# syncdoth/face_mask_inpaint

Measured on AMD Instinct MI355X. Metric: train images/sec at 256x256 bs=8 per GPU (PICNet-ref train step), higher is better.
Workload: dtype f32; 1 GPU; train_reference_fill.py PICNet-ref 256x256 fp32, bs=8 per GPU, synthetic CelebA-HQ-shaped batch + random binary_map (BASELINE configs[1]); global_batch=8, parallelism=dp1

## Files before the change

face_mask_inpaint_amd/_lib.py:

```python
from __future__ import annotations

import ctypes as C
import os

_HERE = os.path.dirname(os.path.abspath(__file__))
LIB_PATH = os.path.join(_HERE, "csrc", "libfmi_hip.so")

c_f = C.c_void_p
i32, i64, f32, f64, vp = C.c_int, C.c_int64, C.c_float, C.c_double, C.c_void_p


class ConvDesc(C.Structure):

    _fields_ = [(n, C.c_int) for n in ("N", "H", "W", "C", "OH", "OW", "K", "x_cstride", "y_cstride", "kh", "kw", "stride", "pad", "pad_mode", "dil")] + [("w3", C.c_void_p), ("x3", C.c_void_p), ("y3", C.c_void_p)]


class WeightEntry(C.Structure):
    _fields_ = [("w", vp), ("u", vp), ("v", vp), ("wf", vp), ("wt", vp), ("sigma", vp), ("rows", i32), ("C", i32), ("taps", i32), ("iters", i32), ("wf3", vp), ("wt3", vp)]


class WeightGradEntry(C.Structure):
    _fields_ = [("w", vp), ("u", vp), ("v", vp), ("sigma", vp), ("dwf", vp), ("dw", vp), ("rows", i32), ("C", i32), ("taps", i32), ("pad_", i32)]


class AdamEntry(C.Structure):
    _fields_ = [("p", vp), ("g", vp), ("m", vp), ("v", vp), ("n", i64)]


class RangerEntry(C.Structure):
    _fields_ = [("p", vp), ("g", vp), ("m", vp), ("v", vp), ("slow", vp), ("row_mean", vp), ("n", i64), ("cols", i64)]


PD = C.POINTER(ConvDesc)

SIGNATURES = {
    "fmi_gemm_f32": [vp, vp, vp, i32, i32, i32, i64, i64, i64, i64, i64, i64, i32, i64, i64, i64, f32, f32, vp, vp],
    "fmi_ssim_valid_f32": [vp, vp, vp, i32, i32, i32, i32, f32, f32, vp, vp, i64, vp],
    "fmi_avgpool2_pad_f32": [vp, vp, i32, i32, i32, i32, i32, vp],
    "fmi_resample_u8": [vp, vp, i32, i32, i32, i32, i32, i32, i32, i32, vp, vp, i32, vp],
    "fmi_gather_u8_i64": [vp, vp, i32, i32, i32, i32, i32, vp, vp, vp],
    "fmi_u8_lut_chw_f32": [vp, vp, vp, i32, i32, i32, i32, vp],
    "fmi_split3_f32": [vp, vp, vp, i64, i32, i32, f32, vp],
    "fmi_split3_colsum_f32": [vp, vp, vp, i64, i32, vp],
    "fmi_merge3_f32": [vp, vp, i64, i32, vp],
    "fmi_conv2d_fwd_f32": [PD, vp, vp, vp, vp, vp, i32, i32, i64, vp],
    "fmi_conv2d_dgrad_f32": [PD, vp, vp, vp, vp, vp, i32, i64, vp],
    "fmi_conv_transpose2d_pair_f32": [PD, vp, vp, i32, vp, vp, vp, vp],
    "fmi_conv_transpose2d_pair_bwd_f32": [PD, vp, vp, i32, vp, vp, vp, vp, vp, vp, vp, vp, vp, i64, vp],
    "fmi_conv2d_pair_fwd_f32": [PD, vp, vp, i32, vp, vp, vp, vp, vp, vp, i32, vp],
    "fmi_conv2d_pair_wgrad_f32": [PD, vp, vp, i32, vp, vp, vp, vp, vp],
    "fmi_conv2d_dgrad_masked_f32": [PD, vp, vp, vp, f32, vp, vp],
    "fmi_conv2d_dgrad_masked_add_f32": [PD, vp, vp, vp, f32, vp, vp, vp],
    "fmi_conv2d_wgrad_f32": [PD, vp, vp, vp, vp, i32, i64, vp],
    "fmi_conv2d_thin_fwd_f32": [PD, vp, vp, vp, vp, vp, i32, vp],
    "fmi_conv2d_thin_dgrad_f32": [PD, vp, vp, vp, vp],
    "fmi_conv2d_thin_input_dgrad_f32": [PD, vp, vp, vp, vp],
    "fmi_conv2d_thin_in_fwd_f32": [PD, vp, vp, vp, vp, vp, i32, vp],
    "fmi_conv2d_thin_in_wgrad_f32": [PD, vp, vp, vp, vp, vp, i64, vp],
    "fmi_conv2d_thin_lrelu_fwd_f32": [PD, vp, f32, vp, vp, vp, i32, vp],
    "fmi_conv2d_thin_lrelu_fwd_bf16": [PD, vp, f32, vp, vp, vp, i32, vp],
    "fmi_conv2d_thin_lrelu_dgrad_f32": [PD, vp, vp, vp, f32, vp, vp],
    "fmi_conv2d_thin_lrelu_wgrad_f32": [PD, vp, f32, vp, vp, vp, vp],
    "fmi_conv2d_thin_wgrad_f32": [PD, vp, vp, vp, vp, vp],
    "fmi_conv2d_thin_lrelu_bwd_f32": [PD, vp, f32, vp, vp, vp, vp, vp, vp, vp, i64, vp],
    "fmi_conv2d_fwd_bf16": [PD, vp, vp, vp, vp, vp, i64, vp],
    "fmi_conv2d_dgrad_bf16": [PD, vp, vp, vp, vp, vp, i64, vp],
    "fmi_conv2d_wgrad_bf16": [PD, vp, vp, vp, vp],
    "fmi_pack_weight_bf16": [vp, vp, i32, i32, i32, vp],
    "fmi_scale_channels_bf16": [vp, vp, vp, i32, i64, i32, vp],
    "fmi_scale_channels_gs_bf16": [vp, vp, vp, vp, i64, i32, i64, i32, vp],
    "fmi_noise_bias_act_bf16": [vp, vp, vp, vp, vp, i64, i32, f32, f32, vp],
    "fmi_noise_bias_act_bwd_bf16": [vp, vp, vp, vp, vp, vp, vp, i64, i64, i32, f32, f32, vp],
    "fmi_upfirdn2d_nhwc_bf16": [vp, vp, vp] + [i32] * 14 + [vp],
    "fmi_styled_out_bwd_bf16": [vp] * 11 + [i64, vp, i32, i64, i32, f32, f32, vp],
    "fmi_conv2d_fwd_act_bf16": [PD, vp, vp, vp, vp, vp, vp, f32, f32, vp, vp],
    "fmi_conv2d_fwd_chan_bf16": [PD, vp, vp, vp, vp, vp, vp, vp, i64, vp],
    "fmi_se_gate_f32": [vp, i32, i64, f32, vp, vp, vp, i32, i32, vp],
    "fmi_irse_tail_bf16": [vp] * 8 + [i32] * 7 + [vp],
    "fmi_irse_stem_bf16": [vp] * 5 + [i64, i32, vp],
    "fmi_conv2d_grouped_fwd_bf16": [PD, i32, i64, vp, vp, vp, f32, vp, vp, vp],
    "fmi_fpn_merge_bf16": [vp] * 4 + [i32] * 6 + [vp],
    "fmi_conv2d_thin_in_fwd_bf16": [PD, vp, vp, vp, f32, vp, vp],
    "fmi_irse_stem_fwd_bf16": [PD] + [vp] * 11,
    "fmi_fpn_merge_in_bf16": [vp] * 3 + [i32] * 6 + [vp],
    "fmi_mask_blend_bf16": [vp] * 4 + [i64, i32, vp],
    "fmi_conv2d_c32_fwd_bf16": [PD, vp, vp, vp, f32, vp, vp],
    "fmi_conv2d_dgrad_relu_bf16": [PD, vp, vp, vp, vp, vp],
    "fmi_vgg_tap_fwd_bf16": [vp, vp, vp, i32, i32, i32, i32, vp],
    "fmi_vgg_tap_bwd_bf16": [vp, vp, vp, vp, i32, i32, i32, i32, vp],
    "fmi_conv2d_thin_input_dgrad_bf16": [PD, vp, vp, vp, vp],
    "fmi_resblock_tail_bf16": [vp] * 5 + [i32] * 5 + [f32, vp],
    "fmi_picnet_stem_tail_bf16": [vp] * 6 + [i32] * 5 + [f32, vp],
    "fmi_guided_attention_fwd_bf16": [vp] * 5 + [i32] * 5 + [vp],
    "fmi_guided_attention_sliced_fwd_bf16": [vp] * 5 + [i32] * 5 + [vp],
    "fmi_blur_act_bf16": [vp, vp, vp] + [i32] * 8 + [vp, vp, vp, vp, f32, f32, i32, vp],
    "fmi_torgb_fwd_bf16": [vp, vp, vp, vp, vp, vp, i32, i64, i32, vp],
    "fmi_torgb_bwd_bf16": [vp, vp, vp, vp, vp, vp, i64, vp, vp, vp, i32, i64, i32, vp],
    "fmi_bias_grad_f32": [vp, i64, i32, i32, vp, vp],
    "fmi_reflect_pad_fold_f32": [vp, vp, i32, i32, i32, i32, i32, vp],
    "fmi_weight_prepare_f32": [vp, i32, vp],
    "fmi_weight_grad_f32": [vp, i32, vp, vp],
    "fmi_softmax_rows_f32": [vp, vp, i64, i32, vp],
    "fmi_softmax_rows_bwd_f32": [vp, vp, vp, i64, i32, vp],
    "fmi_attention_fwd_f32": [vp, vp, vp, vp, vp, vp, i32, i32, i32, i32, i32, vp],
    "fmi_attention_fwd_bf16": [vp] * 6 + [i32] * 5 + [vp],
    "fmi_attention_bwd_f32": [vp] * 12 + [i32] * 5 + [vp],
    "fmi_attention_bwd_prep_bf16": [vp] * 4 + [i32] * 4 + [vp],
    "fmi_attention_bwd_bf16": [vp] * 7 + [i32] * 4 + [vp],
    "fmi_attention_fwd_image_bytes": [i32, i32, i32, i32, i32, C.POINTER(i64)],
    "fmi_attention_fwd_pieces_f32": [vp] * 4 + [i64] + [vp] * 3 + [i32] * 5 + [vp],
    "fmi_attention_bwd_image_bytes": [i32, i32, i32, i32, i32, C.POINTER(i64)],
    "fmi_attention_bwd_pieces_f32": [vp] * 10 + [i64] + [vp] * 3 + [i32] * 5 + [vp],
    "fmi_eltwise_f32": [i32, vp, vp, vp, i64, f32, vp],
    "fmi_axpy_dev_f32": [vp, vp, vp, vp, i64, vp],
    "fmi_dot_f32": [vp, vp, i64, f32, vp, vp],
    "fmi_mask_binarise_i64": [vp, vp, i64, vp],
    "fmi_mask_mul_f32": [vp, vp, vp, i64, i32, i32, vp],
    "fmi_guide_blend_f32": [vp, vp, vp, vp, i64, i32, i32, vp],
    "fmi_guide_blend_bwd_f32": [vp, vp, vp, vp, i64, i32, i32, vp],
    "fmi_vae_sample_f32": [vp, vp, vp, vp, vp, i64, i32, vp],
    "fmi_vae_sample_bwd_f32": [vp, vp, vp, vp, vp, vp, vp, i64, i32, vp],
    "fmi_avgpool_f32": [vp, vp, i32, i32, i32, i32, i32, vp],
    "fmi_avgpool_bwd_f32": [vp, vp, i32, i32, i32, i32, i32, vp],
    "fmi_maxpool2_f32": [vp, vp, i32, i32, i32, i32, vp],
    "fmi_maxpool2_bf16": [vp, vp, i32, i32, i32, i32, vp],
    "fmi_maxpool2_bwd_bf16": [vp, vp, vp, i32, i32, i32, i32, vp],
    "fmi_up2_cat_bf16": [vp, vp, vp, i32, i32, i32, i32, i32, i32, i32, vp],
    "fmi_up2_cat_bwd_bf16": [vp, vp, vp, i32, i32, i32, i32, i32, i32, i32, vp],
    "fmi_head1x1_bf16": [vp, vp, vp, vp, i64, i32, i32, vp],
    "fmi_head1x1_argmax_bf16": [vp, vp, vp, vp, i64, i32, i32, vp],
    "fmi_head1x1_bwd_bf16": [vp, vp, vp, vp, vp, vp, vp, i64, i64, i32, i32, vp],
    "fmi_adaptive_avgpool_f32": [vp, vp, i32, i32, i32, i32, i32, i32, vp],
    "fmi_adaptive_avgpool_bwd_f32": [vp, vp, i32, i32, i32, i32, i32, i32, vp],
    "fmi_maxpool_f32": [vp, vp, vp, i32, i32, i32, i32, i32, i32, vp],
    "fmi_maxpool_bwd_f32": [vp, vp, vp, i32, i32, i32, i32, i32, i32, vp],
    "fmi_argmax_channels_f32": [vp, vp, i64, i32, vp],
    "fmi_image_tail_f32": [vp, vp, vp, vp, i32, i32, f32, f32, vp],
    "fmi_planes_to_u8_f32": [vp, vp, i32, i32, i32, i32, f32, f32, vp],
    "fmi_instnorm_stats_bf16": [vp, vp, vp, i32, i32, i32, f32, vp, i64, vp],
    "fmi_instnorm_apply_bf16": [vp, vp, vp, vp, vp, i32, i32, i32, f32, vp],
    "fmi_instnorm_bwd_reduce_bf16": [vp, vp, vp, vp, vp, vp, i32, i32, i32, f32, vp, i64, vp],
    "fmi_instnorm_bwd_apply_bf16": [vp, vp, vp, vp, vp, vp, vp, vp, vp, vp, i32, i32, i32, f32, vp],
    "fmi_prelu_bf16": [vp, vp, vp, i64, i32, vp],
    "fmi_prelu_bwd_bf16": [vp, vp, vp, vp, vp, vp, i64, i64, i32, vp],
    "fmi_scale_channels_add_bf16": [vp, vp, vp, vp, i32, i64, i32, vp],
    "fmi_add_bf16": [vp, vp, vp, i64, vp],
    "fmi_global_avgpool_bf16": [vp, vp, vp, i64, i32, i64, i32, vp],
    "fmi_add_bcast_bf16": [vp, vp, vp, i32, i64, i32, vp],
    "fmi_add_bcast_f32": [vp, vp, vp, i32, i64, i32, vp],
    "fmi_scale_channels_bwd_f32": [vp, vp, vp, vp, vp, vp, i64, i32, i64, i32, vp],
    "fmi_subsample_bf16": [vp, vp, i32, i32, i32, i32, i32, i32, vp],
    "fmi_scale_channels_add_f32": [vp, vp, vp, vp, i32, i64, i32, vp],
    "fmi_instnorm_bwd_apply_add_f32": [vp, vp, vp, vp, vp, vp, vp, vp, vp, vp, i32, i32, i32, f32, vp],
    "fmi_copy_channels_f32": [vp, vp, i64, i32, i32, i32, i32, i32, vp],
    "fmi_copy_channels_bf16": [vp, vp, i64, i32, i32, i32, i32, i32, vp],
    "fmi_l2norm_rows_f32": [vp, vp, vp, i64, i32, f32, vp],
    "fmi_l2norm_rows_bwd_f32": [vp, vp, vp, vp, i64, i32, f32, vp],
    "fmi_lpips_layer_f32": [vp, vp, vp, vp, i64, i32, f32, vp],
    "fmi_lpips_layer_bwd_f32": [vp, vp, vp, vp, vp, vp, i64, i32, f32, vp],
    "fmi_maxpool2_bwd_f32": [vp, vp, vp, i32, i32, i32, i32, vp],
    "fmi_resize_bilinear_f32": [vp, vp, i32, i32, i32, i32, i32, i32, vp, vp, vp],
    "fmi_resize_bilinear_bwd_f32": [vp, vp, i32, i32, i32, i32, i32, i32, vp, vp],
    "fmi_instnorm_stats_f32": [vp, vp, vp, i32, i32, i32, f32, vp, i64, vp],
    "fmi_batchnorm_running_update_f32": [vp, vp, vp, vp, vp, i32, i64, f32, f32, vp],
    "fmi_batchnorm_running_update_offset_f32": [vp, vp, vp, vp, vp, vp, i32, i64, f32, f32, vp],
    "fmi_instnorm_apply_f32": [vp, vp, vp, vp, vp, i32, i32, i32, f32, vp],
    "fmi_instnorm_bwd_reduce_f32": [vp, vp, vp, vp, vp, vp, i32, i32, i32, f32, vp, i64, vp],
    "fmi_instnorm_bwd_apply_f32": [vp, vp, vp, vp, vp, vp, vp, vp, vp, i32, i32, i32, f32, vp],
    "fmi_reduce_loss_f32": [i32, vp, vp, i64, f32, f32, vp, vp],
    "fmi_reduce_loss_bwd_f32": [i32, vp, vp, i64, f32, f32, vp, vp, vp],
    "fmi_ssim_f32": [vp, vp, vp, i32, i32, i32, i32, i32, vp, vp],
    "fmi_seg_ce_dice_fwd_f32": [vp, vp, i32, i64, i32, f64, vp, vp, vp, i64, vp],
    "fmi_seg_ce_dice_bwd_f32": [vp, vp, i32, i64, i32, f64, vp, vp, vp, vp],
# ... 97 lines not shown
```

face_mask_inpaint_amd/functional.py:

```python
from __future__ import annotations

import ctypes as C
import math
from typing import List, Optional, Sequence, Tuple

import torch

from . import _lib
from ._lib import ConvDesc, FmiError

EW_LRELU, EW_LRELU_BWD, EW_TANH_BWD, EW_ADD, EW_SCALE, EW_AXPY, EW_MUL, EW_RELU_BWD_OUT, EW_SOFTPLUS, EW_SOFTPLUS_BWD, EW_SUB, EW_RSQRT, EW_RSQRT_BWD, EW_SIGMOID, EW_SIGMOID_BWD = range(15)
ACT_NONE, ACT_TANH, ACT_RELU = 0, 1, 2

ATTN_CHUNK_BYTES = 96 * 1024 * 1024

PROFILE = None


class _prof:
    def __init__(self, tag, flops):
        self.tag, self.flops = tag, flops

    def __enter__(self):
        if PROFILE is not None:
# ... 1657 lines not shown
                d, a, prof = _conv_fwd_bf16_pre(hmap, k, 3, 3, 1, 1, " thin-in +relu")
                with prof:
                    lib.conv2d_thin_in_fwd_bf16(C.byref(d), _p(hmap), _p(wf), _p(bias), 0.0, _p(a), _st())
            elif _vgg_fwd_entry(c, k) == "chan":
                a = conv2d_chan_bf16(hmap, wnk, 3, 3, 1, 1, bias=bias, slope=zslope)
            else:
                d, a, prof = _conv_fwd_bf16_pre(hmap, k, 3, 3, 1, 1, " +relu")
                with prof:
                    lib.conv2d_fwd_act_bf16(C.byref(d), _p(hmap), _p(wnk), None, None, None, _p(bias), 0.0, 1.0, _p(a), _st())
            acts.append(a)
            hmap = a
            li += 1
        n, h, w, c = hmap.shape
        tap = torch.empty((n, h, w, c), device=x.device, dtype=torch.float32)
        pooled = torch.empty((n, h // 2, w // 2, c), device=x.device, dtype=BF16) if bi + 1 < len(blocks) else None
        with _prof(f"vgg_tap_fwd_bf16|{n}x{h}x{w}x{c}" + ("" if pooled is None else " +pool"), 0.0):
            lib.vgg_tap_fwd_bf16(_p(hmap), _p(tap), _p(pooled), n, h, w, c, _st())
        taps.append(tap)
        hmap = pooled
    return taps, acts


class _VggTrunkBF16(torch.autograd.Function):

    @staticmethod
    def forward(ctx, x, packs, blocks):
        taps, acts = _vgg_trunk_fwd(x, packs, blocks)
        ctx.save_for_backward(*acts)
        ctx.packs, ctx.blocks = packs, blocks
        ctx.set_materialize_grads(False)
        return tuple(taps)

    @staticmethod
    def backward(ctx, *gtaps):
        lib = _L()
        acts, packs, blocks = ctx.saved_tensors, ctx.packs, ctx.blocks
        first = [sum(blocks[:bi]) for bi in range(len(blocks))]
        gpool = None
        for bi in reversed(range(len(blocks))):
            last = first[bi] + blocks[bi] - 1
            a = acts[last]
            n, h, w, k = a.shape
            if gtaps[bi] is None and gpool is None:
                continue
            gt = torch.zeros((n, h, w, k), device=a.device, dtype=torch.float32) if gtaps[bi] is None else gtaps[bi].contiguous()
            _chk(gt)
            dy = torch.empty_like(a)
            with _prof(f"vgg_tap_bwd_bf16|{n}x{h}x{w}x{k}" + ("" if gpool is None else " +unpool"), 0.0):
                lib.vgg_tap_bwd_bf16(_p(a), _p(gt), _p(gpool), _p(dy), n, h, w, k, _st())
            for li in range(last, first[bi] - 1, -1):
                _wf, wt, _wnk, wck, _bias, _z = packs[li]
                k, c = wt.shape[1], wt.shape[2]
                d, _, _ = conv_desc(n, h, w, c, k, 3, 3, 1, 1)
                flops = 2.0 * dy.numel() * c * 9
                if li == 0:
                    gx = torch.empty((n, h, w, c), device=dy.device, dtype=torch.float32)
                    with _prof(f"conv_dgrad_bf16|{n}x{h}x{w} {c}->{k} k3s1 thin-in", flops):
                        lib.conv2d_thin_input_dgrad_bf16(C.byref(d), _p(dy), _p(wt), _p(gx), _st())
                    return gx, None, None
                dx = torch.empty((n, h, w, c), device=dy.device, dtype=BF16)
                if li > first[bi]:
                    with _prof(f"conv_dgrad_bf16|{n}x{h}x{w} {c}->{k} k3s1 +mask", flops):
                        lib.conv2d_dgrad_relu_bf16(C.byref(d), _p(dy), _p(wck), _p(acts[li - 1]), _p(dx), _st())
                else:
                    with _prof(f"conv_dgrad_bf16|{n}x{h}x{w} {c}->{k} k3s1", flops):
                        lib.conv2d_dgrad_bf16(C.byref(d), _p(dy), _p(wck), None, _p(dx), None, 0, _st())
                dy = dx
            gpool = dy
        return None, None, None


def vgg_trunk_bf16(x, packs, blocks=(2, 2, 3, 3)):
    if x.dim() != 4 or x.shape[3] > 4:
        raise FmiError(f"the bf16 VGG trunk takes an NHWC image with at most 4 channels, got {tuple(x.shape)}")
    vgg_trunk_check_extent(x.shape[1], x.shape[2])
    _chk(x)
    if len(packs) != sum(blocks):
        raise FmiError(f"the bf16 VGG trunk has {sum(blocks)} convolutions, got {len(packs)} packs")
    if torch.is_grad_enabled() and x.requires_grad:
        return list(_VggTrunkBF16.apply(x, packs, tuple(blocks)))
    return _vgg_trunk_fwd(x, packs, tuple(blocks))[0]


class _Resize(torch.autograd.Function):
    @staticmethod
    def forward(ctx, x, oh, ow, mean, std):
        _chk(x, mean, std)
        n, h, w, c = x.shape
        y = torch.empty((n, oh, ow, c), device=x.device, dtype=torch.float32)
        _L().resize_bilinear_f32(_p(x), _p(y), n, h, w, c, oh, ow, _p(mean), _p(std), _st())
        ctx.shape, ctx.std = x.shape, std
        return y

    @staticmethod
    def backward(ctx, g):
        n, h, w, c = ctx.shape
        gx = _zeros(ctx.shape, g.device, torch.float32)
        _L().resize_bilinear_bwd_f32(_p(g.contiguous()), _p(gx), n, h, w, c, g.shape[1], g.shape[2], _p(ctx.std), _st())
        return gx, None, None, None, None


def resize_bilinear(x, oh, ow, mean=None, std=None):
    return _Resize.apply(x, oh, ow, mean, std)


def _norm_ws(device, n, c):
    sums = torch.empty((n, c, 2), device=device, dtype=torch.float64)
    ws = torch.empty(max(1024, n) * c * 2, device=device, dtype=torch.float64)
    return sums, ws


class _InstNormAct(torch.autograd.Function):
    @staticmethod
    def forward(ctx, x, gamma, beta, eps, slope, passthrough=False):
        _chk(x, gamma, beta)
        lib = _L()
        n, h, w, c = x.shape
        sums, ws = _norm_ws(x.device, n, c)
        stats = torch.empty((n, c, 2), device=x.device, dtype=torch.float32)
        lib.instnorm_stats_f32(_p(x), C.c_void_p(sums.data_ptr()), _p(stats), n, h * w, c, eps, C.c_void_p(ws.data_ptr()), ws.numel(), _st())
        y = torch.empty_like(x)
        lib.instnorm_apply_f32(_p(x), _p(stats), _p(gamma), _p(beta), _p(y), n, h * w, c, slope, _st())
        ctx.save_for_backward(x, stats, gamma, beta)
        ctx.slope = slope
        if passthrough:
            return y, x.view_as(x)
        return y

    @staticmethod
    def backward(ctx, g, gpass=None):
        lib = _L()
        x, stats, gamma, beta = ctx.saved_tensors
        if g is None:
            return gpass, None, None, None, None, None
        n, h, w, c = x.shape
        g = g.contiguous()
        red, ws = _norm_ws(x.device, n, c)
        lib.instnorm_bwd_reduce_f32(_p(x), _p(g), _p(stats), _p(gamma), _p(beta), C.c_void_p(red.data_ptr()), n, h * w, c, ctx.slope,
                                    C.c_void_p(ws.data_ptr()), ws.numel(), _st())
        gx = torch.empty_like(x)
        dg = _zeros_like(gamma)
        db = _zeros_like(beta)
        if gpass is not None:
            lib.instnorm_bwd_apply_add_f32(_p(x), _p(g), _p(stats), _p(gamma), _p(beta), C.c_void_p(red.data_ptr()), _p(gpass.contiguous()),
                                           _p(gx), _p(dg), _p(db), n, h * w, c, ctx.slope, _st())
        else:
            lib.instnorm_bwd_apply_f32(_p(x), _p(g), _p(stats), _p(gamma), _p(beta), C.c_void_p(red.data_ptr()), _p(gx), _p(dg), _p(db),
                                       n, h * w, c, ctx.slope, _st())
        return gx, dg, db, None, None, None


def instance_norm_act(x, gamma, beta, eps=1e-5, slope=1.0, passthrough=False):
    return _InstNormAct.apply(x, gamma, beta, eps, slope, passthrough)


class _MaskMul(torch.autograd.Function):
    @staticmethod
    def forward(ctx, x, m, invert):
        _chk(x, m)
        y = torch.empty_like(x)
        c = x.shape[-1]
        _L().mask_mul_f32(_p(x), _p(m), _p(y), x.numel() // c, c, invert, _st())
        ctx.save_for_backward(m)
        ctx.invert = invert
        return y

# ... 1342 lines not shown
```

face_mask_inpaint_amd/modules/loss.py:

```python
from __future__ import annotations

import os

import torch
from torch import nn

from .. import functional as FF
from ..weights import packed
from .pluralistic_model import base_function
from .pluralistic_model.external_function import GANLoss, run_conv

VGG_CFG = [64, 64, "M", 128, 128, "M", 256, 256, 256, "M", 512, 512, 512, "M"]


VGG_DTYPES = {"fp32": torch.float32, "bf16": torch.bfloat16}


def vgg_dtype_from_env():
    name = os.environ.get("FMI_VGG_DTYPE", "fp32")
    if name not in VGG_DTYPES:
        raise FF.FmiError(f"FMI_VGG_DTYPE must be one of {sorted(VGG_DTYPES)}, got {name!r}")
    return VGG_DTYPES[name]


def _vgg16_features(width_div: int = 1) -> nn.Sequential:
    layers, c_in = [], 3
    for v in VGG_CFG:
        if v == "M":
            layers.append(nn.MaxPool2d(kernel_size=2, stride=2))
        else:
            layers += [nn.Conv2d(c_in, v // width_div, kernel_size=3, padding=1), nn.ReLU(inplace=True)]
            c_in = v // width_div
    return nn.Sequential(*layers)


class VGGLoss(torch.nn.Module):
    def __init__(self, width_div: int = 1, feature_dtype=None):
        super().__init__()
        if feature_dtype is None:
            feature_dtype = vgg_dtype_from_env()
        if feature_dtype not in (torch.float32, torch.bfloat16):
            raise FF.FmiError(f"feature_dtype must be torch.float32 or torch.bfloat16, got {feature_dtype}")
        self.feature_dtype = feature_dtype
        try:
            import torchvision

            features = torchvision.models.vgg16(pretrained=True).features
        except Exception:
            features = _vgg16_features(width_div)
        blocks = [features[:4].eval(), features[4:9].eval(), features[9:16].eval(), features[16:23].eval()]
        for bl in blocks:
            for p in bl.parameters():
                p.requires_grad = False
        self.blocks = torch.nn.ModuleList(blocks)
        if feature_dtype == torch.bfloat16:
            FF.vgg_trunk_check_widths([(m.in_channels, m.out_channels) + tuple(m.kernel_size) for bl in blocks for m in bl if isinstance(m, nn.Conv2d)])
        self.register_buffer("mean", torch.tensor([0.485, 0.456, 0.406]).view(1, 3, 1, 1))
        self.register_buffer("std", torch.tensor([0.229, 0.224, 0.225]).view(1, 3, 1, 1))
        self._cache = {}

    def _prepare(self):
        convs = [m for bl in self.blocks for m in bl if isinstance(m, nn.Conv2d)]
        key = tuple((c.weight.data_ptr(), c.weight._version) for c in convs)
        if self._cache.get("key") != key:
            with torch.no_grad():
                pws = FF.prepare_weights([(c.weight, None, None) for c in convs])
                packs16 = FF.vgg_trunk_packs(pws, [c.bias for c in convs]) if self.feature_dtype == torch.bfloat16 else None
            self._cache = {"key": key, "pws": pws, "packs16": packs16}
        for c, pw in zip(convs, self._cache["pws"]):
            object.__setattr__(c, "_fmi_packed", pw)

    def _block(self, bi, x):
        mods = [m for m in self.blocks[bi] if isinstance(m, (nn.MaxPool2d, nn.Conv2d))]
        prev_conv = False
        for i, m in enumerate(mods):
            if isinstance(m, nn.MaxPool2d):
                x = FF.max_pool2(x)
                prev_conv = False
            else:
                next_conv = i + 1 < len(mods) and isinstance(mods[i + 1], nn.Conv2d)
                x = run_conv(m, x, act=FF.ACT_RELU, in_act=("mask", 0.0) if prev_conv else None, skip_act_bwd=next_conv)
                prev_conv = True
        return x

    def _taps16(self, x, y):
        if self.feature_dtype != torch.bfloat16:
            return None, None
        blocks = tuple(sum(isinstance(m, nn.Conv2d) for m in bl) for bl in self.blocks)
        xt = FF.vgg_trunk_bf16(x, self._cache["packs16"], blocks)
        with torch.no_grad():
            yt = FF.vgg_trunk_bf16(y, self._cache["packs16"], blocks)
        return xt, yt

    @staticmethod
    def _input_extent(h, w):
        return (224, 224) if w > 224 else (h, w)

    def _check16(self, h, w):
        if self.feature_dtype == torch.bfloat16:
            FF.vgg_trunk_check_extent(h, w)

    def _input(self, img):
        x = FF.to_nhwc(img)
        n, h, w, c = x.shape
        oh, ow = self._input_extent(h, w)
        return FF.resize_bilinear(x, oh, ow, self.mean.view(3).contiguous(), self.std.view(3).contiguous())

    def forward(self, input, target, lossType="perceptual"):
        self._check16(*self._input_extent(input.shape[2], input.shape[3]))
        self._prepare()
        x = self._input(input)
        with torch.no_grad():
            y = self._input(target)
        loss = 0.0
        xt, yt = self._taps16(x, y)
        for i in range(len(self.blocks)):
            if xt is not None:
                x, y = xt[i], yt[i]
            else:
                x = self._block(i, x)
                with torch.no_grad():
                    y = self._block(i, y)
            n, h, w, c = x.shape
            dim = c * h * w
            if lossType == "perceptual":
                loss = loss + FF.l1_loss(x, y) / dim
            elif lossType == "style":
                gx = FF.gram_matrix(x.view(n, h * w, c))
                gy = FF.gram_matrix(y.view(n, h * w, c))
                loss = loss + FF.l1_loss(gx, gy) / (c * c * dim)
            elif lossType == "contextual" and i == 3:
                loss = loss + FF.contextual_loss(x.view(n, h * w, c), y.view(n, h * w, c)) / dim
        return loss


    def forward_multi(self, triples):
        for t in triples:
            self._check16(*self._input_extent(t[0].shape[2], t[0].shape[3]))
        x = torch.cat([self._input(t[0]) for t in triples], 0)
        with torch.no_grad():
            y = torch.cat([self._input(t[1]) for t in triples], 0)
        return self.forward_multi_prepared(x, y, [t[2] for t in triples])

    def forward_multi_prepared(self, x, y, loss_types):
        self._check16(x.shape[1], x.shape[2])
        self._prepare()
        k = len(loss_types)
        n = x.shape[0] // k
        losses = [0.0] * k
        xt, yt = self._taps16(x, y)
        for i in range(len(self.blocks)):
            if xt is not None:
                x, y = xt[i], yt[i]
            else:
                x = self._block(i, x)
                with torch.no_grad():
                    y = self._block(i, y)
            _, h, w, c = x.shape
            dim = c * h * w
            xparts, yparts = x.split(n, 0), y.split(n, 0)
            for j, lossType in enumerate(loss_types):
                xs, ys = xparts[j], yparts[j]
                if lossType == "perceptual":
                    losses[j] = losses[j] + FF.l1_loss(xs, ys) / dim
                elif lossType == "style":
                    gx = FF.gram_matrix(xs.reshape(n, h * w, c))
                    gy = FF.gram_matrix(ys.reshape(n, h * w, c))
                    losses[j] = losses[j] + FF.l1_loss(gx, gy) / (c * c * dim)
                elif lossType == "contextual" and i == 3:
                    losses[j] = losses[j] + FF.contextual_loss(xs.reshape(n, h * w, c), ys.reshape(n, h * w, c)) / dim
        return losses


class GANOptimizer(nn.Module):

    def __init__(self, optimizer_D, optimizer_G, lambda_g=0.01, debug=False, vgg_width_div: int = 1, vgg_dtype=None):
        super().__init__()
        self.gan_loss = GANLoss("lsgan")
        self.vgg_loss = VGGLoss(vgg_width_div, feature_dtype=vgg_dtype)
        self.debug = debug
        self.optimizer_D = optimizer_D
        self.optimizer_G = optimizer_G
        self.lambda_perc = 0.1
        self.lambda_style = 250
        self.lambda_cx = 1
        self.lambda_g = lambda_g
        self.early_d = None
        self.fused_head = False

    LOSS_TYPES = ("perceptual", "style", "contextual")

    @staticmethod
    def _masked(img, mask, invert):
        return FF.to_nchw(FF.mask_mul(FF.to_nhwc(img), mask.contiguous(), invert))

    def perceptual_loss(self, gt_img, gen_img):
        return self.vgg_loss(gen_img, gt_img, lossType="perceptual")

    def style_loss(self, gen_img, src_img, src_mask):
        return self.vgg_loss(self._masked(gen_img, src_mask, True), src_img, lossType="style")

    def contextual_loss(self, gen_img, ref_img, src_mask):
        return self.vgg_loss(self._masked(gen_img, src_mask, False), self._masked(ref_img, src_mask, False), lossType="contextual")

    def discriminator_loss(self, netD, real, fake):
        D_real_loss = self.gan_loss(netD(real), True, True)
        D_fake_loss = self.gan_loss(netD(fake.detach()), False, True)
        return (D_real_loss + D_fake_loss) * 0.5

    def generator_loss(self, netD, real, fake, freeze=True, l1=None):
        if freeze:
            base_function._freeze(netD)
        D_fake = netD(fake)
        loss_ad_g = self.gan_loss(D_fake, True, False) * self.lambda_g
        loss_l1_g = FF.l1_loss(FF.to_nhwc(fake), FF.to_nhwc(real)) if l1 is None else l1
        return loss_ad_g + loss_l1_g

    def _head(self, src_img, gt_img, ref_img, gen_img, src_mask):
        return FF.gan_image_head(gen_img, gt_img, src_img, ref_img, src_mask, self.vgg_loss.mean, self.vgg_loss.std)

    def __call__(self, discriminator, src_img, gt_img, ref_img, gen_img, src_mask):
        d_params = [p for p in discriminator.parameters() if p.requires_grad]
        for p in d_params:
            p.requires_grad_(False)
        head = self._head(src_img, gt_img, ref_img, gen_img, src_mask) if self.fused_head else None
        try:
            if head is None:
                G_loss = self.generator_loss(discriminator, gt_img, gen_img, freeze=False)
            else:
                G_loss = self.generator_loss(discriminator, gt_img, gen_img, freeze=False, l1=head[2])
        finally:
            for p in d_params:
                p.requires_grad_(True)
        if head is not None:
            perc, sty, cx = self.vgg_loss.forward_multi_prepared(head[0], head[1], self.LOSS_TYPES)
        else:
            perc, sty, cx = self.vgg_loss.forward_multi([
                (gen_img, gt_img, "perceptual"),
                (self._masked(gen_img, src_mask, True), src_img, "style"),
                (self._masked(gen_img, src_mask, False), self._masked(ref_img, src_mask, False), "contextual")])
        perc_loss, style_loss, cx_loss = perc * self.lambda_perc, sty * self.lambda_style, cx * self.lambda_cx
        G_loss = G_loss + perc_loss + style_loss + cx_loss
        early_d = self.early_d if self.early_d is not None else hasattr(self.optimizer_D, "launch")
# ... 68 lines not shown
```

include/fmi_hip.h:

```cpp
#ifndef FMI_HIP_H
#define FMI_HIP_H

#include <stdint.h>

#ifdef __cplusplus
extern "C" {
#endif

typedef enum {
  FMI_OK = 0,
  FMI_ERR_BAD_ARG = 1,
  FMI_ERR_UNSUPPORTED = 2,
  FMI_ERR_LAUNCH = 3
} fmi_status;

const char* fmi_status_string(int status);
int fmi_version(void);
int fmi_set_deterministic(int on);
int fmi_get_deterministic(void);

int fmi_gemm_f32(const float* A, const float* B, float* C, int M, int N, int K,
                 int64_t sa_m, int64_t sa_k, int64_t sb_k, int64_t sb_n, int64_t sc_m, int64_t sc_n,
                 int batch, int64_t sa_b, int64_t sb_b, int64_t sc_b,
                 float alpha, float beta, const float* bias, void* stream);
// ... 343 lines not shown
typedef struct {
  float* p; const float* g; float* m; float* v; float* slow; float* row_mean; int64_t n; int64_t cols;
} fmi_ranger_entry;
int fmi_ranger_step_f32(const fmi_ranger_entry* entries , int count, float lr, float beta1, float beta2, float eps,
                        float weight_decay, float step_size, int rectified, float alpha, int lookahead, void* stream);

int fmi_upfirdn2d_f32(const float* in, const float* kernel, float* out, int major, int in_h, int in_w,
                      int kh, int kw, int up_x, int up_y, int down_x, int down_y,
                      int pad_x0, int pad_x1, int pad_y0, int pad_y1, void* stream);
int fmi_upfirdn2d_bf16(const uint16_t* in, const uint16_t* kernel, uint16_t* out, int major, int in_h, int in_w, int kh, int kw,
                       int up_x, int up_y, int down_x, int down_y, int pad_x0, int pad_x1, int pad_y0, int pad_y1, void* stream);
int fmi_fused_bias_act_f32(const float* x, const float* bias, const float* ref, float* out, int64_t n,
                           int step_b, int size_b, int act, int grad, float alpha, float scale, void* stream);
int fmi_fused_bias_act_bf16(const uint16_t* x, const uint16_t* bias, const uint16_t* ref, uint16_t* out, int64_t n, int step_b,
                            int size_b, int act, int grad, float alpha, float scale, void* stream);
int fmi_bias_grad_nchw_f32(const float* g, int N, int C, int64_t HW, float* dbias, void* stream);
int fmi_bias_grad_nchw_bf16(const void* g, int N, int C, int64_t HW, float* dbias, void* stream);
int fmi_noise_bias_act_f32(const float* x, const float* bias, const float* noise, const float* nw, float* y,
                           int64_t pixels, int C, float alpha, float scale, void* stream);

int fmi_scale_channels_f32(const float* x, const float* s, float* y, int N, int64_t P, int C, void* stream);
int fmi_scale_channels_gs_f32(const float* g, const float* x, float* gs, float* ws, int64_t ws_floats, int N, int64_t P, int C, void* stream);
int fmi_sqsum_last_f32(const float* x, float* out, int64_t rows, int k, void* stream);
int fmi_sqsum_last_bwd_f32(const float* x, const float* g, float* gx, int64_t rows, int k, void* stream);
int fmi_noise_bias_act_bwd_f32(const float* g, const float* y, const float* noise, float* gx, float* gnw,
                               int64_t pixels, int C, float alpha, float scale, void* stream);
int fmi_upfirdn2d_nhwc_f32(const float* in, const float* kernel, float* out, int N, int in_h, int in_w, int C,
                           int kh, int kw, int up_x, int up_y, int down_x, int down_y,
                           int pad_x0, int pad_x1, int pad_y0, int pad_y1, void* stream);

int fmi_prelu_f32(const float* x, const float* a, float* y, int64_t rows, int C, void* stream);
int fmi_prelu_bwd_f32(const float* g, const float* x, const float* a, float* gx, float* ga, float* ws, int64_t ws_floats, int64_t rows,
                      int C, void* stream);
int fmi_subsample_f32(const float* x, float* y, int N, int H, int W, int C, int stride, int backward, void* stream);

int fmi_maxpool2_bf16(const uint16_t* x, uint16_t* y, int N, int H, int W, int C, void* stream);
int fmi_maxpool2_bwd_bf16(const uint16_t* x, const uint16_t* gy, uint16_t* gx, int N, int H, int W, int C, void* stream);
int fmi_up2_cat_bf16(const uint16_t* x1, const uint16_t* skip, uint16_t* y, int N, int h, int w, int C1, int H, int W, int C2, void* stream);
int fmi_up2_cat_bwd_bf16(const uint16_t* g, uint16_t* gskip, uint16_t* gx1, int N, int h, int w, int C1, int H, int W, int C2, void* stream);
int fmi_head1x1_bf16(const uint16_t* x, const float* w, const float* b, float* y, int64_t P, int C, int K, void* stream);
int fmi_head1x1_argmax_bf16(const uint16_t* x, const float* w, const float* b, float* mask, int64_t P, int C, int K, void* stream);
int fmi_head1x1_bwd_bf16(const float* g, const uint16_t* x, const float* w, uint16_t* gx, float* gw, float* gb, double* ws,
                         int64_t ws_doubles, int64_t P, int C, int K, void* stream);

#define FMI_CHAN_COLSUM_ROWS 64
int fmi_conv2d_fwd_chan_bf16(const fmi_conv_desc* d, const uint16_t* x, const uint16_t* wnk, const float* scale, const float* bias,
                             const float* slope, uint16_t* y, float* colsum, int64_t colsum_floats, void* stream);
int fmi_se_gate_f32(const float* part, int rows_per_part, int64_t P, float inv_count, const float* fc1, const float* fc2, float* gates, int N,
                    int C, void* stream);
int fmi_irse_tail_bf16(const uint16_t* r, const float* gate, const uint16_t* sc, const float* next_scale, const float* next_shift, uint16_t* y,
                       uint16_t* z, float* tap, int N, int OH, int OW, int C, int SH, int SW, int sc_stride, void* stream);
int fmi_irse_stem_bf16(const float* x, const float* scale, const float* shift, uint16_t* y, uint16_t* z, int64_t rows, int C, void* stream);

int fmi_conv2d_thin_in_fwd_bf16(const fmi_conv_desc* d, const float* x, const float* wf, const float* bias, float slope, uint16_t* y,
                                void* stream);
int fmi_irse_stem_fwd_bf16(const fmi_conv_desc* d, const float* x, const float* wf, const float* scale, const float* shift, const float* slope,
                           const float* scale0, const float* shift0, uint16_t* y, uint16_t* z, float* a32, void* stream);
int fmi_conv2d_c32_fwd_bf16(const fmi_conv_desc* d, const uint16_t* x, const uint16_t* wnk, const float* bias, float slope, uint16_t* y,
                            void* stream);
int fmi_resblock_tail_bf16(const uint16_t* main_, const uint16_t* shortcut, uint16_t* y_raw, uint16_t* y_act, float* y_f32, int N, int H, int W,
                           int C, int pool, float slope, void* stream);
int fmi_picnet_stem_tail_bf16(const uint16_t* h, const float* img, const float* wb, const float* bias, uint16_t* y_raw, uint16_t* y_act, int N,
                              int H, int W, int C, int K, float slope, void* stream);
int fmi_guided_attention_fwd_bf16_waves(int N, int T);
int fmi_guided_attention_fwd_bf16(const uint16_t* q, const uint16_t* src, const uint16_t* ref, const float* mask, uint16_t* out, int N, int T,
                                  int D, int C, int waves, void* stream);
int fmi_guided_attention_sliced_fwd_bf16(const uint16_t* q, const uint16_t* src, const uint16_t* ref, const float* mask, uint16_t* out, int N,
                                         int T, int D, int C, int waves, void* stream);

#define FMI_STYLE_SKINNY_ROWS 128
int fmi_conv2d_grouped_fwd_bf16(const fmi_conv_desc* d, int G, int64_t x_group_off, const uint16_t* x, const uint16_t* wnk,
                                const float* bias, float slope, uint16_t* y16, float* y32, void* stream);
int fmi_fpn_merge_bf16(const float* lateral, const float* coarse, float* p32, uint16_t* p16, int N, int H, int W, int CH, int CW, int C,
                       void* stream);
int fmi_fpn_merge_in_bf16(const uint16_t* lateral, const uint16_t* coarse, uint16_t* p16, int N, int H, int W, int CH, int CW, int C,
                          void* stream);
int fmi_mask_blend_bf16(const uint16_t* r, const uint16_t* c, const float* m, uint16_t* y, int64_t rows, int C, void* stream);

int fmi_conv2d_dgrad_relu_bf16(const fmi_conv_desc* d, const uint16_t* dy, const uint16_t* wck, const uint16_t* a_in, uint16_t* dx, void* stream);
int fmi_vgg_tap_fwd_bf16(const uint16_t* a, float* tap, uint16_t* pooled, int N, int H, int W, int C, void* stream);
int fmi_vgg_tap_bwd_bf16(const uint16_t* a, const float* gtap, const uint16_t* gpool, uint16_t* dy, int N, int H, int W, int C, void* stream);
int fmi_conv2d_thin_input_dgrad_bf16(const fmi_conv_desc* d, const uint16_t* dy16, const float* wt, float* dx, void* stream);

#ifdef __cplusplus
}
#endif
#endif
```

Before: 108.7 images/s.

## Add fused fp32 VGG trunk with pooled taps and sliced-gradient backward

Adds an fp32 VGG perceptual-loss trunk path. It runs the image and target through the convolutions in one merged batch and fuses max-pooling with emitting the split-bf16 pieces the next convolution consumes. The backward pass uses a custom kernel that combines the ReLU mask, the unpooling via argmax, and per-slice tap gradients, and it can write split pieces directly so the dgrad convolution may skip reading fp32. This cuts kernel launches and intermediate memory passes in the loss network, at the cost of a larger custom autograd path that needs 3x3 convolutions and channel counts that are multiples of four.

```diff
diff --git a/face_mask_inpaint_amd/_lib.py b/face_mask_inpaint_amd/_lib.py
--- a/face_mask_inpaint_amd/_lib.py
+++ b/face_mask_inpaint_amd/_lib.py
@@ -89,6 +89,8 @@
     "fmi_vgg_tap_fwd_bf16": [vp, vp, vp, i32, i32, i32, i32, vp],
     "fmi_vgg_tap_bwd_bf16": [vp, vp, vp, vp, i32, i32, i32, i32, vp],
     "fmi_conv2d_thin_input_dgrad_bf16": [PD, vp, vp, vp, vp],
+    "fmi_vgg_tap_fwd_f32": [vp, vp, vp, i32, i32, i32, i32, vp],
+    "fmi_vgg_tap_bwd_f32": [vp, vp, i32, i32, vp, vp, vp, i32, i32, i32, i32, vp],
     "fmi_resblock_tail_bf16": [vp] * 5 + [i32] * 5 + [f32, vp],
     "fmi_picnet_stem_tail_bf16": [vp] * 6 + [i32] * 5 + [f32, vp],
     "fmi_guided_attention_fwd_bf16": [vp] * 5 + [i32] * 5 + [vp],
diff --git a/face_mask_inpaint_amd/csrc/vgg_f32.hip b/face_mask_inpaint_amd/csrc/vgg_f32.hip
--- /dev/null
+++ b/face_mask_inpaint_amd/csrc/vgg_f32.hip
@@ -0,0 +1,163 @@
+#include "common.h"
+#include "x6.h"
+
+#define VT_MAX_SLICES 4
+
+__device__ __forceinline__ void vt_pieces(uint16_t* __restrict__ x3, int64_t i, const float4& a, const float4& b) {
+  uint32_t w[3][4];
+  split3_pair(a.x, a.y, w[0][0], w[1][0], w[2][0]);
+  split3_pair(a.z, a.w, w[0][1], w[1][1], w[2][1]);
+  split3_pair(b.x, b.y, w[0][2], w[1][2], w[2][2]);
+  split3_pair(b.z, b.w, w[0][3], w[1][3], w[2][3]);
+  uint16_t* q = x3 + (i >> 1) * 48 + (i & 1) * 8;
+#pragma unroll
+  for (int pc = 0; pc < 3; ++pc) *reinterpret_cast<uint4*>(q + pc * 16) = make_uint4(w[pc][0], w[pc][1], w[pc][2], w[pc][3]);
+}
+
+__device__ __forceinline__ float vt_max4(float p0, float p1, float p2, float p3) { return fmaxf(fmaxf(fmaxf(p0, p1), p2), p3); }
+
+template <int V>
+__global__ void __launch_bounds__(256) vgg_tap_fwd_f32_kernel(const float4* __restrict__ a, float4* __restrict__ pooled, uint16_t* __restrict__ pooled3,
+                                                              int H, int W, int CV, int64_t total) {
+  const int OH = H >> 1, OW = W >> 1;
+  const int64_t right = (int64_t)CV * V, down = (int64_t)W * CV * V;
+  for (int64_t i = (int64_t)blockIdx.x * 256 + threadIdx.x; i < total; i += (int64_t)gridDim.x * 256) {
+    const int c = (int)(i % CV);
+    int64_t r = i / CV;
+    const int ox = (int)(r % OW);
+    r /= OW;
+    const int oy = (int)(r % OH);
+    const int64_t n = r / OH;
+    const int64_t o = (((n * H + oy * 2) * W + ox * 2) * CV + c) * V;
+    float4 m[V];
+#pragma unroll
+    for (int e = 0; e < V; ++e) {
+      const float4 p0 = a[o + e], p1 = a[o + right + e], p2 = a[o + down + e], p3 = a[o + down + right + e];
+      m[e] = make_float4(vt_max4(p0.x, p1.x, p2.x, p3.x), vt_max4(p0.y, p1.y, p2.y, p3.y), vt_max4(p0.z, p1.z, p2.z, p3.z),
+                         vt_max4(p0.w, p1.w, p2.w, p3.w));
+      pooled[i * V + e] = m[e];
+    }
+    if constexpr (V == 2) vt_pieces(pooled3, i, m[0], m[1]);
+  }
+}
+
+__device__ __forceinline__ uint32_t vt_arg(float v0, float v1, float v2, float v3) {
+  uint32_t arg = 0;
+  float m = v0;
+  if (v1 > m) { m = v1; arg = 1; }
+  if (v2 > m) { m = v2; arg = 2; }
+  if (v3 > m) { m = v3; arg = 3; }
+  return arg;
+}
+template <int V, bool ADD>
+__device__ __forceinline__ float vt_dy(float g, float gp, uint32_t posm, uint32_t argm, int k, int ch) {
+  if (ADD) g = g + (((argm >> (2 * ch)) & 3u) == (uint32_t)k ? gp : 0.f);
+  return ((posm >> (k * 4 * V + ch)) & 1u) ? g : 0.f;
+}
+
+template <int V, bool ADD>
+__global__ void __launch_bounds__(256) vgg_tap_bwd_f32_kernel(const float4* __restrict__ a, const float4* __restrict__ g0, const float4* __restrict__ g1,
+                                                              const float4* __restrict__ g2, const float4* __restrict__ g3, int per_slice,
+                                                              int64_t slice_f4, const float4* __restrict__ gpool, float4* __restrict__ dy,
+                                                              uint16_t* __restrict__ dy3, int H, int W, int CV, int64_t total) {
+  const int OH = H >> 1, OW = W >> 1, WH = (H + 1) >> 1, WW = (W + 1) >> 1;
+  const int64_t right = (int64_t)CV * V, down = (int64_t)W * CV * V;
+  const float4 z4 = make_float4(0.f, 0.f, 0.f, 0.f);
+  for (int64_t i = (int64_t)blockIdx.x * 256 + threadIdx.x; i < total; i += (int64_t)gridDim.x * 256) {
+    const int c = (int)(i % CV);
+    int64_t r = i / CV;
+    const int wx = (int)(r % WW);
+    r /= WW;
+    const int wy = (int)(r % WH);
+    const int64_t n = r / WH;
+    const bool has_r = wx * 2 + 1 < W, has_d = wy * 2 + 1 < H;
+    const bool pool = ADD && wy < OH && wx < OW;
+    const int64_t o = (((n * H + wy * 2) * W + wx * 2) * CV + c) * V;
+    const int s = (int)(n / per_slice);
+    const float4* gsl = s == 0 ? g0 : s == 1 ? g1 : s == 2 ? g2 : g3;
+    const int64_t go = o - (int64_t)s * slice_f4;
+    const int64_t off[4] = {0, right, down, down + right};
+    const bool has[4] = {true, has_r, has_d, has_r && has_d};
+    uint32_t posm = 0, argm = 0;
+    float4 gp[V];
+#pragma unroll
+    for (int e = 0; e < V; ++e) {
+      float4 p[4];
+#pragma unroll
+      for (int k = 0; k < 4; ++k) {
+        p[k] = has[k] ? a[o + off[k] + e] : z4;
+        posm |= ((p[k].x > 0.f ? 1u : 0u) | (p[k].y > 0.f ? 2u : 0u) | (p[k].z > 0.f ? 4u : 0u) | (p[k].w > 0.f ? 8u : 0u)) << (k * 4 * V + e * 4);
+      }
+      gp[e] = z4;
+      if (pool) {
+        gp[e] = gpool[((((n * OH + wy) * OW + wx) * CV) + c) * V + e];
+        argm |= (vt_arg(p[0].x, p[1].x, p[2].x, p[3].x) | vt_arg(p[0].y, p[1].y, p[2].y, p[3].y) << 2 | vt_arg(p[0].z, p[1].z, p[2].z, p[3].z) << 4 |
+                 vt_arg(p[0].w, p[1].w, p[2].w, p[3].w) << 6) << (e * 8);
+      }
+    }
+#pragma unroll 1
+    for (int k = 0; k < 4; ++k) {
+      if (((k & 1) && !has_r) || ((k & 2) && !has_d)) continue;
+      const int64_t offk = (k & 1 ? right : 0) + (k & 2 ? down : 0);
+      float4 out[V];
+#pragma unroll
+      for (int e = 0; e < V; ++e) {
+        const float4 g = gsl ? gsl[go + offk + e] : z4;
+        out[e] = make_float4(vt_dy<V, ADD>(g.x, gp[e].x, posm, argm, k, e * 4), vt_dy<V, ADD>(g.y, gp[e].y, posm, argm, k, e * 4 + 1),
+                             vt_dy<V, ADD>(g.z, gp[e].z, posm, argm, k, e * 4 + 2), vt_dy<V, ADD>(g.w, gp[e].w, posm, argm, k, e * 4 + 3));
+        if (dy) dy[o + offk + e] = out[e];
+      }
+      if constexpr (V == 2) {
+        if (dy3) vt_pieces(dy3, (o + offk) >> 1, out[0], out[1]);
+      }
+    }
+  }
+}
+
+extern "C" int fmi_vgg_tap_fwd_f32(const float* a, float* pooled, void* pooled3, int N, int H, int W, int C, void* stream) {
+  if (!a || !pooled || N <= 0 || H < 2 || W < 2 || C <= 0) return FMI_ERR_BAD_ARG;
+  if (C % 4 != 0 || (pooled3 && C % 16 != 0) || !fmi_al16(a) || !fmi_al16(pooled) || !fmi_al16(pooled3)) return FMI_ERR_UNSUPPORTED;
+  hipStream_t st = (hipStream_t)stream;
+  const int64_t windows = (int64_t)N * (H / 2) * (W / 2);
+  if (pooled3) {
+    const int64_t total = windows * (C / 8);
+    hipLaunchKernelGGL(vgg_tap_fwd_f32_kernel<2>, dim3(fmi_bw_grid(total, 256)), dim3(256), 0, st, (const float4*)a, (float4*)pooled,
+                       (uint16_t*)pooled3, H, W, C / 8, total);
+  } else {
+    const int64_t total = windows * (C / 4);
+    hipLaunchKernelGGL(vgg_tap_fwd_f32_kernel<1>, dim3(fmi_bw_grid(total, 256)), dim3(256), 0, st, (const float4*)a, (float4*)pooled,
+                       (uint16_t*)nullptr, H, W, C / 4, total);
+  }
+  return fmi_launch_status();
+}
+
+template <int V>
+static void vt_launch_bwd(const float* a, const float4* const (&gs)[VT_MAX_SLICES], int per_slice, const float* gpool, float* dy, void* dy3, int N, int H, int W, int C,
+                          hipStream_t st) {
+  const int CV = C / (4 * V);
+  const int64_t total = (int64_t)N * ((H + 1) / 2) * ((W + 1) / 2) * CV;
+  const int64_t slice_f4 = (int64_t)per_slice * H * W * (C / 4);
+  const dim3 grid(fmi_bw_grid(total, 256)), block(256);
+  if (gpool)
+    hipLaunchKernelGGL((vgg_tap_bwd_f32_kernel<V, true>), grid, block, 0, st, (const float4*)a, gs[0], gs[1], gs[2], gs[3], per_slice, slice_f4, (const float4*)gpool,
+                       (float4*)dy, (uint16_t*)dy3, H, W, CV, total);
+  else
+    hipLaunchKernelGGL((vgg_tap_bwd_f32_kernel<V, false>), grid, block, 0, st, (const float4*)a, gs[0], gs[1], gs[2], gs[3], per_slice, slice_f4, (const float4*)nullptr,
+                       (float4*)dy, (uint16_t*)dy3, H, W, CV, total);
+}
+
+extern "C" int fmi_vgg_tap_bwd_f32(const float* a, const float* const* gslice, int nslice, int rows_per_slice, const float* gpool, float* dy,
+                                   void* dy3, int N, int H, int W, int C, void* stream) {
+  if (!a || !gslice || (!dy && !dy3) || N <= 0 || H <= 0 || W <= 0 || C <= 0) return FMI_ERR_BAD_ARG;
+  if (nslice < 1 || nslice > VT_MAX_SLICES || rows_per_slice < 1 || (int64_t)nslice * rows_per_slice != N) return FMI_ERR_BAD_ARG;
+  if (gpool && (H < 2 || W < 2)) return FMI_ERR_BAD_ARG;
+  if (C % 4 != 0 || (dy3 && C % 16 != 0) || !fmi_al16(a) || !fmi_al16(gpool) || !fmi_al16(dy) || !fmi_al16(dy3)) return FMI_ERR_UNSUPPORTED;
+  const float4* gs[VT_MAX_SLICES] = {nullptr, nullptr, nullptr, nullptr};
+  for (int s = 0; s < nslice; ++s) {
+    if (!fmi_al16(gslice[s])) return FMI_ERR_UNSUPPORTED;
+    gs[s] = (const float4*)gslice[s];
+  }
+  if (dy3) vt_launch_bwd<2>(a, gs, rows_per_slice, gpool, dy, dy3, N, H, W, C, (hipStream_t)stream);
+  else vt_launch_bwd<1>(a, gs, rows_per_slice, gpool, dy, dy3, N, H, W, C, (hipStream_t)stream);
+  return fmi_launch_status();
+}
diff --git a/face_mask_inpaint_amd/functional.py b/face_mask_inpaint_amd/functional.py
--- a/face_mask_inpaint_amd/functional.py
+++ b/face_mask_inpaint_amd/functional.py
@@ -1763,6 +1763,153 @@
     return _vgg_trunk_fwd(x, packs, tuple(blocks))[0]
 
 
+_PLAN_FLAGS_P3 = 0x1 | 0x2 | 0x4 | 0x20 | 0x40 | 0x80 | 0x100
+_PLAN_FLAG_MASK = 0x1000
+
+
+def _dgrad_reads_f32(d, masked: bool) -> bool:
+    out = (C.c_int * 44)()
+    rc = _L().conv2d_f32_plan(C.byref(d), 1, _PLAN_FLAGS_P3 | (_PLAN_FLAG_MASK if masked else 0), out)
+    if rc != 0 or out[2] != 0 or not 1 <= out[1] <= 4:
+        return True
+    return any(out[4 + 10 * p] not in (3, 6) for p in range(out[1]))
+
+
+def vgg_trunk_f32_ok(pws: Sequence[PackedWeight], blocks) -> bool:
+    ends = [sum(blocks[:bi + 1]) - 1 for bi in range(len(blocks))]
+    return all(pw.kh == 3 and pw.kw == 3 for pw in pws) and all(pws[e].rows % 4 == 0 for e in ends)
+
+
+def _vgg_conv_fwd_f32(hmap, h3, pw, bias):
+    n, h, w, c = hmap.shape
+    k = pw.wf.shape[2]
+    d, _, _ = conv_desc(n, h, w, c, k, 3, 3, 1, 1, w3=pw.w3[0], x3=h3)
+    a = torch.empty((n, h, w, k), device=hmap.device, dtype=torch.float32)
+    with _prof(f"conv_fwd|{n}x{h}x{w} {c}->{k} k3s1", 2.0 * n * h * w * k * c * 9):
+        _L().conv2d_fwd_f32(C.byref(d), _p(hmap), _p(pw.wf), _p(bias), None, _p(a), ACT_RELU, 1, 0, _st())
+    return a
+
+
+def _vgg_wants3(pw, pixels, adjoint=False):
+    if adjoint:
+        return pw.w3[1] is not None and pw.rows % 16 == 0 and p3_wanted(pixels, pw.rows, pw.C, 9)
+    return pw.w3[0] is not None and pw.C % 16 == 0 and p3_wanted(pixels, pw.C, pw.rows, 9)
+
+
+def _vgg_trunk_fwd_f32(x, convs, blocks):
+    lib = _L()
+    acts, li, hmap, h3 = [], 0, x, None
+    for bi, nconv in enumerate(blocks):
+        for _ in range(nconv):
+            pw, bias = convs[li]
+            n, h, w, c = hmap.shape
+            src = hmap if h3 is None and _vgg_wants3(pw, n * h * w) else None
+            if src is not None:
+                h3 = p3_of(src)
+            hmap, h3 = _vgg_conv_fwd_f32(hmap, h3, pw, bias), None
+            if src is not None:
+                src._fmi_p3 = None
+            acts.append(hmap)
+            li += 1
+        if bi + 1 < len(blocks):
+            n, h, w, c = hmap.shape
+            pooled = torch.empty((n, h // 2, w // 2, c), device=x.device, dtype=torch.float32)
+            if _vgg_wants3(convs[li][0], pooled.numel() // c):
+                h3 = torch.empty(pooled.numel() * 3, device=x.device, dtype=torch.bfloat16)
+            with _prof(f"vgg_tap_fwd_f32|{n}x{h}x{w}x{c}" + ("" if h3 is None else " +pieces"), 0.0):
+                lib.vgg_tap_fwd_f32(_p(hmap), _p(pooled), None if h3 is None else C.c_void_p(h3.data_ptr()), n, h, w, c, _st())
+            hmap = pooled
+    return acts
+
+
+def _vgg_trunk_f32_taps(x, y, convs, blocks, nslice, merge):
+    n = x.shape[0]
+    if y is not None and merge:
+        acts = _vgg_trunk_fwd_f32(torch.cat([x, y], 0), convs, blocks)
+        yacts = [a[n:] for a in acts]
+    else:
+        acts = _vgg_trunk_fwd_f32(x, convs, blocks)
+        yacts = _vgg_trunk_fwd_f32(y, convs, blocks) if y is not None else None
+    ends = [sum(blocks[:bi + 1]) - 1 for bi in range(len(blocks))]
+    xs = [s for e in ends for s in (acts[e][:n].split(n // nslice, 0) if nslice > 1 else (acts[e][:n],))]
+    return acts, xs, ([] if yacts is None else [yacts[e] for e in ends])
+
+
+class _VggTrunkF32(torch.autograd.Function):
+
+    @staticmethod
+    def forward(ctx, x, y, convs, blocks, nslice, merge):
+        acts, xs, ys = _vgg_trunk_f32_taps(x, y, convs, blocks, nslice, merge)
+        ctx.save_for_backward(*acts)
+        ctx.convs, ctx.blocks, ctx.nslice, ctx.n = convs, blocks, nslice, x.shape[0]
+        ctx.set_materialize_grads(False)
+        ctx.mark_non_differentiable(*ys)
+        return tuple(xs) + tuple(ys)
+
+    @staticmethod
+    def backward(ctx, *grads):
+        lib = _L()
+        acts, convs, blocks, ns, n = ctx.saved_tensors, ctx.convs, ctx.blocks, ctx.nslice, ctx.n
+        first = [sum(blocks[:bi]) for bi in range(len(blocks))]
+        gpool = None
+        for bi in reversed(range(len(blocks))):
+            last = first[bi] + blocks[bi] - 1
+            a = acts[last][:n]
+            _, h, w, k = a.shape
+            gs = [None if g is None else g.contiguous() for g in grads[bi * ns:(bi + 1) * ns]]
+            if gpool is None and all(g is None for g in gs):
+                continue
+            _chk(*gs)
+            if any(g is not None and g.data_ptr() % 16 for g in gs):
+                gs = [torch.cat([torch.zeros_like(a[:n // ns]) if g is None else g for g in gs], 0)]
+            pw = convs[last][0]
+            want3 = _vgg_wants3(pw, n * h * w, adjoint=True)
+            dy3 = torch.empty(a.numel() * 3, device=a.device, dtype=torch.bfloat16) if want3 else None
+            d, _, _ = conv_desc(n, h, w, pw.C, k, 3, 3, 1, 1, w3=pw.w3[1], x3=dy3)
+            gy = torch.empty_like(a) if (dy3 is None or _dgrad_reads_f32(d, blocks[bi] > 1)) else None
+            ptrs = (C.c_void_p * len(gs))(*[None if g is None else g.data_ptr() for g in gs])
+            with _prof(f"vgg_tap_bwd_f32|{n}x{h}x{w}x{k}" + ("" if gpool is None else " +unpool") + ("" if dy3 is None else " +pieces"), 0.0):
+                lib.vgg_tap_bwd_f32(_p(a), ptrs, len(gs), n // len(gs), _p(gpool), _p(gy), None if dy3 is None else C.c_void_p(dy3.data_ptr()),
+                                    n, h, w, k, _st())
+            gy3 = dy3
+            for li in range(last, first[bi] - 1, -1):
+                pw = convs[li][0]
+                k, c = pw.rows, pw.C
+                if li < last:
+                    gy3 = p3_of(gy) if _vgg_wants3(pw, n * h * w, adjoint=True) else None
+                    d, _, _ = conv_desc(n, h, w, c, k, 3, 3, 1, 1, w3=pw.w3[1], x3=gy3)
+                gx = torch.empty((n, h, w, c), device=a.device, dtype=torch.float32)
+                with _prof(f"conv_dgrad|{n}x{h}x{w} {c}->{k} k3s1", 2.0 * n * h * w * k * c * 9):
+                    if li > first[bi]:
+                        lib.conv2d_dgrad_masked_f32(C.byref(d), _p(a if gy is None else gy), _p(pw.wt), _p(acts[li - 1][:n]), 0.0, _p(gx), _st())
+                    else:
+                        lib.conv2d_dgrad_f32(C.byref(d), _p(a if gy is None else gy), _p(pw.wt), None, None, _p(gx), 1, 0, _st())
+                gy = gx
+            gpool = gy
+        return gpool, None, None, None, None, None
+
+
+def vgg_trunk_f32(x, y, convs, blocks=(2, 2, 3, 3), nslice=1, merge=True):
+    _chk(x, y)
+    blocks = tuple(blocks)
+    if len(convs) != sum(blocks):
+        raise FmiError(f"the fp32 VGG trunk has {sum(blocks)} convolutions, got {len(convs)}")
+    if not vgg_trunk_f32_ok([pw for pw, _ in convs], blocks):
+        raise FmiError("the fp32 VGG trunk needs 3 x 3 convolutions and tap widths that are multiples of 4")
+    if not 1 <= nslice <= 4 or x.shape[0] % nslice or (y is not None and y.shape != x.shape):
+        raise FmiError(f"the fp32 VGG trunk: batch {x.shape[0]} in {nslice} slices (1..4), target {None if y is None else tuple(y.shape)}")
+    merge = bool(merge) and y is not None
+    nb = len(blocks)
+    if torch.is_grad_enabled() and x.requires_grad:
+        out = _VggTrunkF32.apply(x, y, tuple(convs), blocks, nslice, merge)
+    else:
+        with torch.no_grad():
+            _, xs, ys = _vgg_trunk_f32_taps(x, y, tuple(convs), blocks, nslice, merge)
+        out = tuple(xs) + tuple(ys)
+    xs = [out[bi] if nslice == 1 else tuple(out[bi * nslice:(bi + 1) * nslice]) for bi in range(nb)]
+    return xs, list(out[nb * nslice:])
+
+
 class _Resize(torch.autograd.Function):
     @staticmethod
     def forward(ctx, x, oh, ow, mean, std):
diff --git a/face_mask_inpaint_amd/modules/loss.py b/face_mask_inpaint_amd/modules/loss.py
--- a/face_mask_inpaint_amd/modules/loss.py
+++ b/face_mask_inpaint_amd/modules/loss.py
@@ -83,10 +83,14 @@
                 prev_conv = True
         return x
 
-    def _taps16(self, x, y):
+    def _taps16(self, x, y, nslice=1):
+        blocks = tuple(sum(isinstance(m, nn.Conv2d) for m in bl) for bl in self.blocks)
         if self.feature_dtype != torch.bfloat16:
-            return None, None
-        blocks = tuple(sum(isinstance(m, nn.Conv2d) for m in bl) for bl in self.blocks)
+            convs = [m for bl in self.blocks for m in bl if isinstance(m, nn.Conv2d)]
+            pws = self._cache["pws"]
+            if not (x.is_cuda and x.dtype == torch.float32 and FF.vgg_trunk_f32_ok(pws, blocks)) or x.shape[0] % nslice or nslice > 4:
+                return None, None
+            return FF.vgg_trunk_f32(x, y, [(pw, c.bias) for pw, c in zip(pws, convs)], blocks, nslice=nslice)
         xt = FF.vgg_trunk_bf16(x, self._cache["packs16"], blocks)
         with torch.no_grad():
             yt = FF.vgg_trunk_bf16(y, self._cache["packs16"], blocks)
@@ -148,7 +152,8 @@
         k = len(loss_types)
         n = x.shape[0] // k
         losses = [0.0] * k
-        xt, yt = self._taps16(x, y)
+        xt, yt = self._taps16(x, y, nslice=k)
+        sliced = xt is not None and k > 1 and isinstance(xt[0], tuple)
         for i in range(len(self.blocks)):
             if xt is not None:
                 x, y = xt[i], yt[i]
@@ -156,9 +161,9 @@
                 x = self._block(i, x)
                 with torch.no_grad():
                     y = self._block(i, y)
-            _, h, w, c = x.shape
+            xparts, yparts = x if sliced else x.split(n, 0), y.split(n, 0)
+            _, h, w, c = y.shape
             dim = c * h * w
-            xparts, yparts = x.split(n, 0), y.split(n, 0)
             for j, lossType in enumerate(loss_types):
                 xs, ys = xparts[j], yparts[j]
                 if lossType == "perceptual":
diff --git a/include/fmi_hip.h b/include/fmi_hip.h
--- a/include/fmi_hip.h
+++ b/include/fmi_hip.h
@@ -449,6 +449,10 @@
 int fmi_vgg_tap_bwd_bf16(const uint16_t* a, const float* gtap, const uint16_t* gpool, uint16_t* dy, int N, int H, int W, int C, void* stream);
 int fmi_conv2d_thin_input_dgrad_bf16(const fmi_conv_desc* d, const uint16_t* dy16, const float* wt, float* dx, void* stream);
 
+int fmi_vgg_tap_fwd_f32(const float* a, float* pooled, void* pooled3, int N, int H, int W, int C, void* stream);
+int fmi_vgg_tap_bwd_f32(const float* a, const float* const* gslice, int nslice, int rows_per_slice, const float* gpool, float* dy, void* dy3,
+                        int N, int H, int W, int C, void* stream);
+
 #ifdef __cplusplus
 }
 #endif
```

Result: faster. 112.2 images/s (median of 6 runs) (+3.3%).
